# NikhilMukraj/spiking-neural-networks

Measured on AMD Instinct MI355X. Metric: neuron-steps/sec, higher is better.
Workload: dtype f32; 1 GPU; 256x256 Izhikevich lattice, dense gap-junction connectivity (all-to-all, x != y), dt=0.1, weights U[0.5,1.5]; neurons=65536, parallelism=single GPU

## Files before the change

### spiking-neural-networks_amd/csrc/snn_network.hip

```cpp
#include "snn_network_state.hpp"
#include "snn_network_step.hpp"
#include "snn_network_exchange.hpp"
#include "snn_network_verify.hpp"
#include "snn_network_graph.hpp"
#include "snn_network_edge_history.hpp"
#include "snn_network_peaks.hpp"

extern "C" {

int snn_abi_version(void) ABI_TRY { return SNN_ABI_VERSION; } ABI_CATCH
const char *snn_custom_model(void) ABI_TRY { return custom::TYPE_NAME; } ABI_CATCH_PTR
const char *snn_custom_spike_train(void) ABI_TRY { return custom_st::TYPE_NAME; } ABI_CATCH_PTR
const char *snn_custom_refractoriness(void) ABI_TRY { return custom_refr::TYPE_NAME; } ABI_CATCH_PTR
const char *snn_custom_neurotransmitter_kinetics(void) ABI_TRY { return custom_nt::TYPE_NAME; } ABI_CATCH_PTR
const char *snn_custom_receptor_kinetics(void) ABI_TRY { return custom_rc::TYPE_NAME; } ABI_CATCH_PTR
const char *snn_custom_receptors(void) ABI_TRY { return custom_receptors::TYPE_NAME; } ABI_CATCH_PTR
const char *snn_last_error(void) ABI_TRY { return g_last_error.c_str(); } ABI_CATCH_PTR

int snn_network_create(int device, int neuron_model, int nt_kinetics, int receptor_kinetics,
                       int spike_train_model, snn_network_t **out) ABI_TRY
{
    if (!out) return fail(SNN_ERR_BAD_ARG, "out is null");
    *out = nullptr;
    const bool custom_ok = SNN_HAVE_CUSTOM_NEURON && neuron_model == SNN_MODEL_CUSTOM;
    const bool custom_st_ok = SNN_HAVE_CUSTOM_SPIKE_TRAIN && spike_train_model == SNN_ST_CUSTOM;
    const bool custom_nt_ok = SNN_HAVE_CUSTOM_NT && nt_kinetics == SNN_NT_CUSTOM;
    const bool custom_rc_ok = SNN_HAVE_CUSTOM_RC && receptor_kinetics == SNN_RC_CUSTOM;
    if (((neuron_model < 0 || neuron_model > 8) && !custom_ok) || ((nt_kinetics < 0 || nt_kinetics > 3) && !custom_nt_ok) ||
        ((receptor_kinetics < 0 || receptor_kinetics > 2) && !custom_rc_ok) ||
        ((spike_train_model < 0 || spike_train_model > 4) && !custom_st_ok))
        return fail(SNN_ERR_BAD_ARG, "unknown model / kinetics selector");
    int ndev = 0;
    if (hipGetDeviceCount(&ndev) != hipSuccess || ndev <= 0)
        return fail(SNN_ERR_GET_DEVICE, "no HIP device visible");
    if (device < 0 || device >= ndev) return fail(SNN_ERR_GET_DEVICE, "device ordinal out of range");
    HIP_TRY(hipSetDevice(device), SNN_ERR_GET_DEVICE);
    snn_network *net = new snn_network();
    net->device = device;
    for (const OptionRow &r : OPTION_TABLE)
        if (const char *e = r.source != OPTION_ONLY ? getenv(option_env_name(r).c_str()) : nullptr) net->opt.*r.member = option_from_env(r, e);
    net->model = neuron_model; net->nt_kind = nt_kinetics; net->rc_kind = receptor_kinetics;
    net->st_kind = spike_train_model;
    if (const char *e = getenv("SNN_AMD_W24")) net->w24_enabled = !(e[0] == '0' && e[1] == '\0');
    if (hipStreamCreateWithFlags(&net->own_stream, hipStreamNonBlocking) != hipSuccess) {
        delete net;
        return fail(SNN_ERR_QUEUE, "hipStreamCreate failed");
    }
    net->stream = net->own_stream;
    *out = net;
    return SNN_OK;
}
ABI_CATCH

int snn_network_destroy(snn_network_t *net) ABI_TRY
{
    if (!net) return SNN_OK;
    (void)hipSetDevice(net->device);
    if (net->stream) (void)hipStreamSynchronize(net->stream);
    for (auto &e : net->ev_pool) { (void)hipEventDestroy(e.first); (void)hipEventDestroy(e.second); }
    for (auto &e : net->ev_pool_pl) { (void)hipEventDestroy(e.first); (void)hipEventDestroy(e.second); }
    if (net->comm_stream) { (void)hipStreamSynchronize(net->comm_stream); (void)hipStreamDestroy(net->comm_stream); }
    if (net->ev_packed) (void)hipEventDestroy(net->ev_packed);
    if (net->ev_exchanged) (void)hipEventDestroy(net->ev_exchanged);
    if (net->own_stream) (void)hipStreamDestroy(net->own_stream);
    delete net;
    return SNN_OK;
}
ABI_CATCH

static int add_lattice_impl(snn_network_t *net, uint32_t id, uint32_t rows, uint32_t cols, bool st)
{
    if (!net) return fail(SNN_ERR_BAD_ARG, "net is null");
    if (net->finalized) return fail(SNN_ERR_BAD_STATE, "lattices cannot be added after finalize");
    if (find_lattice(net, id))
        return fail(SNN_ERR_BAD_ARG, "lattice id " + std::to_string(id) + " already present");
    if (st && net->st_kind == SNN_ST_NONE) return fail(SNN_ERR_BAD_STATE, "network was created without a spike-train model");
    if ((uint64_t)rows * cols > 0x7FFFFFFFull) return fail(SNN_ERR_DIM_MISMATCH, "lattice too large");
    LatticeInfo l{id, rows, cols, 0, rows * cols, 0, st};
    (st ? net->st_lattices : net->lattices).push_back(l);
    return SNN_OK;
}

int snn_network_add_lattice(snn_network_t *net, uint32_t id, uint32_t rows, uint32_t cols) ABI_TRY
{
    return add_lattice_impl(net, id, rows, cols, false);
}
ABI_CATCH
int snn_network_add_spike_train_lattice(snn_network_t *net, uint32_t id, uint32_t rows, uint32_t cols) ABI_TRY
{
    return add_lattice_impl(net, id, rows, cols, true);
}
ABI_CATCH

static int finalize_impl(snn_network_t *net, int kind, uint32_t post_begin, uint32_t post_end, uint32_t n_shards,
                         uint32_t stride, uint32_t shard_index)
{
    const bool whole = kind == 0;
    if (!net) return fail(SNN_ERR_BAD_ARG, "net is null");
    if (net->finalized) return fail(SNN_ERR_BAD_STATE, "already finalized");
    HIP_TRY(hipSetDevice(net->device), SNN_ERR_GET_DEVICE);
    auto by_id = [](const LatticeInfo &a, const LatticeInfo &b) { return a.id < b.id; };
    std::sort(net->lattices.begin(), net->lattices.end(), by_id);
    std::sort(net->st_lattices.begin(), net->st_lattices.end(), by_id);
    uint64_t off = 0;
    uint32_t slot = 0;
    for (auto &l : net->lattices) { l.first = (uint32_t)off; l.slot = slot++; off += l.count; }
    net->nn = (uint32_t)off;
    slot = 0;
    for (auto &l : net->st_lattices) { l.first = (uint32_t)off; l.slot = slot++; off += l.count; }
    if (off > 0x7FFFFFFFull) return fail(SNN_ERR_DIM_MISMATCH, "network too large");
    net->n_tot = (uint32_t)off;
    net->nc = net->n_tot - net->nn;
    net->n_pad = std::max<uint32_t>(256, round_up(net->nn, 256));
    net->c_pad = std::max<uint32_t>(256, round_up(net->nc, 256));
    if (whole) {
        net->q0 = 0; net->q1 = net->nn;
    } else if (kind == 1) {
        if (post_begin > post_end || post_end > net->nn) return fail(SNN_ERR_DIM_MISMATCH, "shard range outside the population");
        if (stride == 0 || stride % 64 != 0 || n_shards == 0 || (uint64_t)stride * n_shards < net->nn)
            return fail(SNN_ERR_BAD_ARG, "shard stride must be a multiple of 64 covering the population");
        net->q0 = post_begin; net->q1 = post_end;
        net->sharded = true;
        net->n_shards = n_shards; net->shard_stride = stride; net->shard_index = shard_index;
        net->n_pad = std::max<uint32_t>(net->n_pad, round_up(stride * n_shards, 256));
    } else {
        net->q0 = 0; net->q1 = 0;
// ... 891 lines not shown
ABI_CATCH

int snn_set_spike_train_clock(snn_network_t *net, uint32_t id, uint64_t clock) ABI_TRY
{
    if (!net) return fail(SNN_ERR_BAD_ARG, "net is null");
    if (!net->finalized) return fail(SNN_ERR_BAD_STATE, "network not finalized");
    const LatticeInfo *l = find_lattice(net, id);
    if (!l || !l->spike_train) return fail(SNN_ERR_BAD_ARG, "no such spike-train lattice");
    if (clock > 0x7FFFFFFFull) return fail(SNN_ERR_BAD_ARG, "the clock must fit the firing times' 31 bits");
    HIP_TRY(hipSetDevice(net->device), SNN_ERR_GET_DEVICE);
    TRY(end_run(net));
    net->st_clock[l->slot] = (long long)clock;
    return SNN_OK;
}
ABI_CATCH

int snn_get_spike_train_clock(snn_network_t *net, uint32_t id, uint64_t *clock) ABI_TRY
{
    if (!net || !clock) return fail(SNN_ERR_BAD_ARG, "null argument");
    if (!net->finalized) return fail(SNN_ERR_BAD_STATE, "network not finalized");
    const LatticeInfo *l = find_lattice(net, id);
    if (!l || !l->spike_train) return fail(SNN_ERR_BAD_ARG, "no such spike-train lattice");
    HIP_TRY(hipSetDevice(net->device), SNN_ERR_GET_DEVICE);
    TRY(end_run(net));
    *clock = (uint64_t)net->st_clock[l->slot];
    return SNN_OK;
}
ABI_CATCH

const char *snn_debug_verify_report(snn_network_t *net) ABI_TRY { return net ? net->verify_text.c_str() : ""; } ABI_CATCH_PTR

int snn_debug_fail_alloc_at(int64_t n, uint64_t *allocations_so_far) ABI_TRY
{
    AllocFault &f = alloc_fault();
    if (allocations_so_far) *allocations_so_far = f.seen.load(std::memory_order_relaxed);
    f.countdown.store(n > 0 ? n : 0, std::memory_order_relaxed);
    return SNN_OK;
}
ABI_CATCH

int snn_debug_set_host_allocator(snn_host_alloc_fn alloc, snn_host_release_fn release) ABI_TRY
{
    static HostAllocHooks hooks;
    if ((alloc == nullptr) != (release == nullptr)) return fail(SNN_ERR_BAD_ARG, "both functions or none");
    if (!alloc) { host_alloc_hooks().store(nullptr, std::memory_order_release); return SNN_OK; }
    hooks.alloc = alloc; hooks.release = release;
    host_alloc_hooks().store(&hooks, std::memory_order_release);
    return SNN_OK;
}
ABI_CATCH

int snn_debug_checkpoint(snn_network_t *net, int restore) ABI_TRY
{
    if (!net) return fail(SNN_ERR_BAD_ARG, "net is null");
    if (!net->finalized) return fail(SNN_ERR_BAD_STATE, "network not finalized");
    HIP_TRY(hipSetDevice(net->device), SNN_ERR_GET_DEVICE);
    TRY(end_run(net));
    if (restore) net->img_stale = net->img_stale_direct = true;
    if (restore) w24_invalidate(net);
    auto &cp = net->checkpoint;
    hvec<std::pair<void *, size_t>> arrays;
    for (const auto &r : net->registry)
        if (!r.scratch) arrays.emplace_back(r.mem.get(), r.bytes);
    if (net->csr_w) arrays.emplace_back(net->csr_w, (size_t)net->sell_entries * 4);
    if (net->trace) arrays.emplace_back(net->trace, std::max<size_t>(trace_elems(net), 64) * 4);
    for (void *m : {(void *)net->pending, (void *)net->edge_counter})
        if (m) arrays.emplace_back(m, std::max<size_t>(trace_elems(net), 64) * 4);
    size_t total = 0;
    for (const auto &a : arrays) total += a.second;
    if (total > ((size_t)256 << 20)) return fail(SNN_ERR_BAD_STATE, "checkpoints are for small handles (256 MiB of device state at most)");
    const size_t peak_words = (net->want_peaks && net->pk_raster) ? (size_t)net->cur.hist_steps * (net->n_pad / 64) : 0;
    if (!restore) {
        hvec<unsigned long long> peak_rows(peak_words);
        if (peak_words) HIP_TRY(copy_sync(net, peak_rows.data(), net->pk_raster, peak_words * 8, hipMemcpyDeviceToHost), SNN_ERR_BUFFER_READ);
        cp.peak_rows.swap(peak_rows);
        cp.peak_epoch = net->pk_epoch;
        cp.arrays.clear();
        for (const auto &a : arrays) {
            cp.arrays.emplace_back(a.first, hvec<uint8_t>(a.second));
            HIP_TRY(hipMemcpyAsync(cp.arrays.back().second.data(), a.first, a.second, hipMemcpyDeviceToHost, net->stream), SNN_ERR_BUFFER_READ);
        }
        HIP_TRY(hipStreamSynchronize(net->stream), SNN_ERR_WAIT);
        cp.st_clock = net->st_clock; cp.cur = net->cur; cp.cache = net->cache; cp.persistent_run = net->opt.persistent_run;
        cp.valid = true;
        return SNN_OK;
    }
    if (!cp.valid) return fail(SNN_ERR_BAD_STATE, "no checkpoint was taken");
    if (cp.peak_epoch != net->pk_epoch) return fail(SNN_ERR_BAD_STATE, "the handle's structure changed since the checkpoint (peak records switched)");
    std::map<void *, size_t> current(arrays.begin(), arrays.end());
    for (const auto &a : cp.arrays) {
        const auto it = current.find(a.first);
        if (it == current.end() || it->second != a.second.size())
            return fail(SNN_ERR_BAD_STATE, "the handle's structure changed since the checkpoint");
    }
    for (const auto &a : cp.arrays)
        HIP_TRY(hipMemcpyAsync(a.first, a.second.data(), a.second.size(), hipMemcpyHostToDevice, net->stream), SNN_ERR_BUFFER_WRITE);
    HIP_TRY(hipStreamSynchronize(net->stream), SNN_ERR_WAIT);
    if (!cp.peak_rows.empty())
        HIP_TRY(copy_sync(net, net->pk_raster, cp.peak_rows.data(), cp.peak_rows.size() * 8, hipMemcpyHostToDevice), SNN_ERR_BUFFER_WRITE);
    net->st_clock = cp.st_clock; net->cur = cp.cur; net->cache = cp.cache; net->opt.persistent_run = cp.persistent_run;
    net->stdp_pending = false; net->stdp_pending_rows_only = false; net->rstdp_pending = false; net->reward_since_defer = false;
    net->cells_stepped = false; net->local_inputs_done = false; net->run_tag = 1;
    if (net->run_granules) {
        HIP_TRY(hipMemsetAsync(net->run_granules, 0, RUN_GRANULE_WORDS * 8, net->stream), SNN_ERR_BUFFER_WRITE);
        HIP_TRY(hipMemsetAsync(net->run_partials, 0, RUN_PARTIAL_WORDS * 8, net->stream), SNN_ERR_BUFFER_WRITE);
        HIP_TRY(hipStreamSynchronize(net->stream), SNN_ERR_WAIT);
    }
    return SNN_OK;
}
ABI_CATCH

extern "C++" {
namespace {
int run_steps(snn_network *net, uint64_t iterations)
{
    uint64_t it = 0;
    if (iterations >= 4 && net->external_stream && run_resident_shape(net)) net->stat.run_external_stream += 1;
    while (iterations - it >= 4 && run_resident_applies(net)) {
        const uint64_t chunk = std::min<uint64_t>(iterations - it, std::max<uint32_t>(4u, net->opt.run_resident_chunk_steps));
        const RunCursors saved{net->cur, net->stat.run, net->ev_used};
        TRY(run_snapshot(net, false));
        TRY(launch_run_resident(net, chunk, it));
        if (!net->opt.persistent_run) break;
        HIP_TRY(hipStreamSynchronize(net->stream), SNN_ERR_WAIT);
        if (net->run_failed && net->run_failed[0]) {
            net->run_failed[0] = 0u;
            TRY(run_snapshot(net, true));
            HIP_TRY(hipMemsetAsync(net->run_granules, 0, RUN_GRANULE_WORDS * 8, net->stream), SNN_ERR_BUFFER_WRITE);
            HIP_TRY(hipMemsetAsync(net->run_partials, 0, RUN_PARTIAL_WORDS * 8, net->stream), SNN_ERR_BUFFER_WRITE);
            net->run_tag = 1;
            net->cur = saved.cur; net->stat.run = saved.run; net->ev_used = saved.ev_used;
            net->cache.shadow_valid = false;
            net->cache.view_dirty = true;
            net->opt.persistent_run = 0;
            net->stat.run_fallbacks += 1;
            break;
        }
        it += chunk;
    }
    for (; it < iterations; ++it) {
        if (net->nn) TRY(step_begin(net));
        TRY(step_end(net));
        if (net->profile && (net->ev_used >= 8192 || net->ev_used_pl >= 8192)) TRY(collect_profile(net));
    }
    return SNN_OK;
}
}
}

int snn_run(snn_network_t *net, uint64_t iterations) ABI_TRY
{
    if (!net) return fail(SNN_ERR_BAD_ARG, "net is null");
    if (!net->finalized) return fail(SNN_ERR_BAD_STATE, "network not finalized");
    if (net->n_shards > 1) return fail(SNN_ERR_BAD_STATE, "sharded handles are stepped with snn_step_begin/end or snn_run_sharded");
    if (iterations == 0 || net->n_tot == 0) return SNN_OK;
    if (!net->electrical && !net->chemical) return SNN_OK;
    HIP_TRY(hipSetDevice(net->device), SNN_ERR_GET_DEVICE);
    TRY(begin_run(net, iterations));
    TRY(verify_applies(net) ? run_verified(net, iterations) : run_steps(net, iterations));
    return end_run(net, true);
}
ABI_CATCH

int snn_step_begin_local(snn_network_t *net) ABI_TRY
{
    if (!net) return fail(SNN_ERR_BAD_ARG, "net is null");
    if (!net->finalized) return fail(SNN_ERR_BAD_STATE, "network not finalized");
    if (!net->electrical && !net->chemical) return SNN_OK;
    HIP_TRY(hipSetDevice(net->device), SNN_ERR_GET_DEVICE);
    TRY(begin_run(net, 1));
    if (net->interior_pending) return step_interior(net);
    if (net->nn && !net->csr && !net->any_plasticity && !net->any_modulation && !net->drive_threshold && !net->local_inputs_done) {
        TRY(launch_inputs(net, INPUTS_LOCAL));
        net->local_inputs_done = true;
    }
    return SNN_OK;
}
ABI_CATCH

// ... 830 lines not shown
```

### spiking-neural-networks_amd/csrc/snn_network_state.hpp

```cpp
#pragma once
#include <hip/hip_runtime.h>

#include <algorithm>
#include <atomic>
#include <chrono>
#include <cmath>
#include <cstdint>
#include <cstdio>
#include <cstdlib>
#include <cstring>
#include <map>
#include <memory>
#include <new>
#include <stdexcept>
#include <string>
#include <utility>
#include <vector>

#include "../../include/snn_amd.h"
#include "snn_kernels_connect.hpp"
#include "snn_kernels_connect_csr.hpp"
#include "snn_kernels_csr.hpp"
#include "snn_kernels_dense_step.hpp"
#include "snn_kernels_edge_history.hpp"
// ... 205 lines not shown
    bool reward_since_defer = false;

    uint32_t nn = 0, nc = 0, n_tot = 0, n_pad = 0, c_pad = 0;
    uint32_t q0 = 0, q1 = 0, n_loc = 0, ld = 0, n_chunks = 0;
    XLayout xl{0};
    bool sharded = false;
    uint32_t n_shards = 1, shard_index = 0, shard_stride = 0;
    bool block_mode = false;
    hvec<uint32_t> lattice_slab;
    hvec<std::pair<uint32_t, uint32_t>> ranges;
    uint32_t n_owned = 0;
    hvec<uint32_t> owned_local_host;
    hvec<uint32_t> local_row_host;
    dev_ptr<uint32_t> own_block_dev, local_row_dev;
    dev_ptr<unsigned long long> own_mask_dev;
    RowMap rowmap{};
    bool x_dirty = true;
    bool x_agreed = false;
    bool refresh_agreed = false;
    int x_mode = SNN_EXCHANGE_ALLGATHER;
    uint32_t x_planes = 0, x_plane_id[WIRE_MAX_PLANES] = {0, 0, 0, 0};
    uint64_t x_block_words = 0;
    uint32_t *wire = nullptr;
    size_t wire_words = 0;
    hvec<hvec<uint32_t>> halo_need, halo_send;
    bool halo_committed = false;
    dev_ptr<uint32_t> halo_send_buf, halo_recv_buf, halo_send_idx, halo_recv_idx;
    hvec<uint64_t> x_send_off, x_send_words, x_recv_off, x_recv_words;
    dev_ptr<uint32_t> seg_count_dev[2], seg_first_dev[2];
    dev_ptr<uint64_t> seg_offset_dev[2], seg_loff_dev[2];
    uint32_t seg_n[2] = {0, 0}, seg_max[2] = {0, 0};
    dev_ptr<uint32_t> csr_border_dev, csr_interior_dev;
    uint32_t n_border = 0, n_interior = 0;
    dev_ptr<uint32_t> pack_ptr_dev, pack_segoff_dev, pack_count_dev, pack_index_dev;
    uint32_t recv_total = 0, send_bitmap_words = 0;
    bool send_bits_clean = true;
    bool update_packed = false;
    bool step_packed = false;
    bool interior_pending = false;
    dev_ptr<uint32_t> halo_send_buf2, halo_recv_buf2;
    dev_ptr<uint32_t> csr_plan_direct, halo_word_dev;
    bool direct_capable = false;
    bool peer_capable = false;
    bool direct_run = false;
    int hx_par = 0;
    bool stamp_pending = false;
    bool tail_done = false;
    dev_ptr<unsigned long long> p2p_recv[2];
    dev_ptr<uint32_t> p2p_flags;
    dev_ptr<uint32_t> p2p_done_blocks;
    pinned_ptr<uint32_t> p2p_failed;
    dev_ptr<uint32_t> agree_words_dev;
    uint32_t agree_words_cap = 0;
    uint64_t p2p_recv_words = 0;
    struct P2pPeer { uint64_t recv[2] = {0, 0}, flags = 0, recv_offset = 0; bool set = false; };
    hvec<P2pPeer> p2p_peers;
    dev_ptr<unsigned long long *> p2p_dst_dev[2];
    dev_ptr<uint32_t> p2p_peer_dev;
    dev_ptr<uint32_t *> p2p_signal_dev;
    uint32_t p2p_n_signal = 0;
    bool p2p_connected = false;
    hvec<dev_ptr<void>> p2p_retired;
    bool peer_run = false;
    uint32_t p2p_epoch = 0;
    hipStream_t comm_stream = nullptr;
    hipEvent_t ev_packed = nullptr, ev_exchanged = nullptr;

    struct Registered { dev_ptr<void> mem; size_t bytes; bool scratch; };
    hvec<Registered> registry;
    uint64_t registry_generation = 0;
    bool csr = false;
    uint64_t nnz = 0;
    dev_ptr<uint32_t> csr_ptr, csr_pre, csr_post, csr_t_ptr, csr_t_edge;
    dev_ptr<uint32_t> csr_row_len, csr_edge_slot;
    dev_ptr<float> csr_w;
    uint64_t sell_entries = 0;
    hvec<uint32_t> edge_slot_host;
    float *W = nullptr;
    dev_ptr<uint32_t> w24, w24_range;
    uint32_t w24_base = 0;
    bool w24_valid = false;
    bool w24_refused = false;
    bool w24_enabled = true;
    float *xbuf = nullptr;
    float *part_i = nullptr, *part_t = nullptr;
    uint32_t *n_in = nullptr, *tcount = nullptr;
    NeuronArrays na{};
    CellArrays ca{};
    uint32_t *lattice_slot = nullptr;
    float *stdp_dev = nullptr;
    uint32_t *plast_dev = nullptr;
    uint32_t *spike_list = nullptr, *spike_count = nullptr;
    hvec<uint32_t> cell_list_host;
    dev_ptr<uint32_t> cell_list_dev;
    uint32_t n_cells_listed = 0;
    dev_ptr<uint32_t> csr_plan;
    dev_ptr<uint32_t> csr_img_hdr, csr_plan_win;
    dev_ptr<uint4> csr_img_rec;
    uint64_t img_records = 0, img_staged_slices = 0;
    bool img_stale = true;
    dev_ptr<uint32_t> csr_img_hdr_direct, csr_plan_win_direct;
    dev_ptr<uint4> csr_img_rec_direct;
    uint64_t img_staged_slices_direct = 0;
    bool img_stale_direct = true;
    hvec<uint32_t> sell_pre_host, slice_ptr_host;
    uint2 *cell_view[2] = {nullptr, nullptr};
    bool cells_stepped = false;
    UniformTable *uni_neuron = nullptr, *uni_cell = nullptr;
    unsigned long long *run_granules = nullptr;
    unsigned long long *run_partials = nullptr;
    uint32_t run_tag = 1;
    float *run_w_out = nullptr;
    pinned_ptr<uint32_t> run_failed;
    uint32_t run_probed_grid = 0;
    CopyEntry *snap_table = nullptr;
    uint32_t *snap_buf = nullptr;
    uint32_t snap_entries = 0, snap_max_words = 0;
    uint64_t snap_registry_seen = 0;
    size_t snap_words = 0;
    hvec<CopyEntry> snap_table_host;
    size_t verify_words = 0;
    uint32_t *verify_buf = nullptr;
    dev_ptr<uint32_t> verify_report;
    pinned_ptr<char> copy_stage;
    dev_ptr<uint32_t> verify_third;
    size_t verify_third_words = 0;
    dev_ptr<char> verify_big;
    size_t verify_big_bytes = 0;
    uint64_t snap_generation = 0;
    std::string verify_text;
    struct Checkpoint {
        bool valid = false;
        hvec<std::pair<void *, hvec<uint8_t>>> arrays;
        hvec<long long> st_clock;
        Cursors cur;
        CacheState cache;
        uint32_t persistent_run = 1;
        hvec<unsigned long long> peak_rows;
        uint64_t peak_epoch = 0;
    } checkpoint;
    unsigned long long *run_timing = nullptr;
    unsigned long long run_timing_last[4] = {0, 0, 0, 0};
    uint32_t run_timing_steps = 0;
    bool stdp_pending = false;
    bool stdp_pending_rows_only = false;
    uint32_t *stdp_rowbits = nullptr;
    uint32_t *stdp_flag = nullptr;
    float *stdp_dcol = nullptr, *stdp_drow = nullptr;
    uint32_t dcol_stride = 0;
    long long *st_clock_dev = nullptr;
    pinned_ptr<long long> st_clock_pinned;
    bool run_active = false;
    float *shadow[2] = {nullptr, nullptr};
    uint32_t *tile_done = nullptr;
    uint32_t tile_done_len = 0;
    bool local_inputs_done = false;

    std::map<std::string, Attr> neuron_attrs, cell_attrs;

    int want_vhist = 0, want_raster = 0;
    int want_avg = 0, want_eeg = 0, want_counts = 0;
    hvec<int> want_whist;
    hvec<dev_ptr<float>> whist;
    bool any_whist = false;
    hvec<uint32_t> eh_slot;
    uint32_t eh_n1 = 0, eh_n2 = 0, eh_first2 = 0, eh_ld = 0;
    dev_ptr<uint32_t> eh_pre, eh_post;
    dev_ptr<unsigned long long> eh_offset;
    dev_ptr<float> eh_hist;
    hvec<uint2> pk_cfg_host;
    dev_ptr<uint2> pk_cfg;
    bool want_peaks = false;
    float *pk_prev = nullptr;
    uint32_t *pk_left = nullptr;
    dev_ptr<unsigned long long> pk_raster;
    uint64_t pk_epoch = 0;
    float eeg_ref = 0.007f, eeg_dist = 0.8f, eeg_cond = 251.0f;
    dev_ptr<float> summ_avg, summ_eeg;
    uint32_t *spike_counts = nullptr, *lat_first_dev = nullptr, *lat_count_dev = nullptr;
    uint64_t hist_cap = 0;
    hvec<hvec<float>> preset_host;
    dev_ptr<float> preset_times_dev;
    uint32_t hist_every = 1;
    dev_ptr<float> vhist, st_vhist;
    dev_ptr<unsigned long long> raster;

    uint64_t drive_seed = 0;
    uint32_t drive_threshold = 0;
    float drive_voltage = 0.0f;
    hvec<std::pair<hipEvent_t, hipEvent_t>> ev_pool_pl;
    size_t ev_used_pl = 0;
    uint64_t prof_launches_pl = 0;
    double prof_ms_pl = 0.0;
    int profile = 0;
    hvec<std::pair<hipEvent_t, hipEvent_t>> ev_pool;
    hvec<int> ev_counts;
    size_t ev_used = 0;
    uint64_t prof_launches = 0;
    double prof_ms = 0.0;
};

namespace {
static_assert(Options{}.run_resident_spin_limit == RUN_RESIDENT_SPIN_LIMIT, "snn_options.hpp restates the kernel header's default");

struct StatRow { const char *name; uint64_t (*read)(const snn_network &); };
#define STAT(field) [](const snn_network &n) -> uint64_t { return n.field; }
const StatRow STAT_TABLE[] = {
    {"persistent_run_launches", STAT(stat.run.launches)},
    {"persistent_run_steps", STAT(stat.run.steps)},
    {"persistent_run_stdp_steps", STAT(stat.run.stdp_steps)},
    {"persistent_run_fallbacks", STAT(stat.run_fallbacks)},
    {"persistent_run_external_stream", STAT(stat.run_external_stream)},
    {"halo_direct_steps", STAT(stat.direct_steps)},
    {"halo_peer_steps", STAT(stat.peer_steps)},
    {"steps_dense_one_launch", STAT(stat.steps_dense_one_launch)},
    {"steps_dense_close", STAT(stat.steps_dense_close)},
// ... 749 lines not shown
```

### spiking-neural-networks_amd/csrc/snn_network_step.hpp

```cpp
#pragma once
#include "snn_dispatch.hpp"
#include "snn_network_state.hpp"

namespace {

enum ProfilePool { PROFILE_GRAPH_PASS, PROFILE_PLASTICITY };
int profile_open(snn_network *net, ProfilePool which, int passes, hipEvent_t *e1)
{
    *e1 = nullptr;
    if (!net->profile) return SNN_OK;
    auto &pool = which == PROFILE_PLASTICITY ? net->ev_pool_pl : net->ev_pool;
    size_t &used = which == PROFILE_PLASTICITY ? net->ev_used_pl : net->ev_used;
    if (used == pool.size()) {
        hipEvent_t x, y;
        HIP_TRY(hipEventCreate(&x), SNN_ERR_QUEUE);
        HIP_TRY(hipEventCreate(&y), SNN_ERR_QUEUE);
        pool.emplace_back(x, y);
    }
    if (which == PROFILE_GRAPH_PASS) {
        net->ev_counts.resize(pool.size(), 1);
        net->ev_counts[used] = passes;
    }
    const auto ev = pool[used++];
    *e1 = ev.second;
// ... 443 lines not shown
    if (net->n_loc == 0 || net->nn == 0) { net->stdp_pending_rows_only = false; return SNN_OK; }
    StdpArgs a = stdp_args(net);
    const unsigned sy = 64;
    if (net->stdp_pending_rows_only) {
        net->stdp_pending_rows_only = false;
    } else {
        hipLaunchKernelGGL(k_stdp_apply_columns, dim3((net->n_tot + 255) / 256, sy), dim3(256), 0, net->stream, a);
        HIP_TRY(hipGetLastError(), SNN_ERR_QUEUE);
    }
    hipLaunchKernelGGL(k_stdp_apply_rows, dim3((net->n_loc + 255) / 256, sy), dim3(256), 0, net->stream, a);
    HIP_TRY(hipGetLastError(), SNN_ERR_QUEUE);
    return SNN_OK;
}

int flush_rstdp(snn_network *net)
{
    if (!net->rstdp_pending) return SNN_OK;
    net->rstdp_pending = false;
    return launch_rstdp_pass(net, net->reward_since_defer ? RM_DOPAMINE_BEFORE : RM_DOPAMINE);
}

int time_input_pass(snn_network *net, float *ms)
{
    *ms = 0.0f;
    hipEvent_t e0 = nullptr, e1 = nullptr;
    if (hipEventCreate(&e0) != hipSuccess || hipEventCreate(&e1) != hipSuccess) return fail(SNN_ERR_QUEUE, "hipEventCreate failed");
    const size_t bytes = (size_t)net->n_tot * net->ld * 4;
    const int passes = bytes < ((size_t)4 << 30) ? 8 : 1;
    int rc = launch_inputs(net);
    if (rc == SNN_OK && hipEventRecord(e0, net->stream) != hipSuccess) rc = fail(SNN_ERR_QUEUE, "hipEventRecord failed");
    for (int i = 0; i < passes && rc == SNN_OK; ++i) rc = launch_inputs(net);
    if (rc == SNN_OK && (hipEventRecord(e1, net->stream) != hipSuccess || hipEventSynchronize(e1) != hipSuccess ||
                         hipEventElapsedTime(ms, e0, e1) != hipSuccess))
        rc = fail(SNN_ERR_WAIT, "placement timing failed");
    *ms /= (float)passes;
    (void)hipEventDestroy(e0);
    (void)hipEventDestroy(e1);
    return rc;
}

int choose_matrix_placement(snn_network *net)
{
    const size_t count = net->csr ? 0 : wcount(net->n_tot, net->ld);
    const size_t bytes = count * sizeof(float);
    if (bytes >= ((size_t)1 << 30) && net->n_loc) {
        const int prof = net->profile;
        net->profile = 0;
        float best_ms = 0.0f;
        int rc = time_input_pass(net, &best_ms);
        hvec<dev_ptr<void>> losers;
        for (int cand = 0; cand < 4 && rc == SNN_OK; ++cand) {
            size_t free_b = 0, total_b = 0;
            dev_ptr<void> b;
            if (hipMemGetInfo(&free_b, &total_b) != hipSuccess || free_b < bytes + (bytes >> 2) ||
                alloc_streamed(&b, bytes) != hipSuccess)
                break;
            float *a = net->W;
            float ms_b = 0.0f;
            net->W = static_cast<float *>(b.get());
            rc = time_input_pass(net, &ms_b);
            if (getenv("SNN_DEBUG_PLACEMENT"))
                fprintf(stderr, "[snn] matrix placement: held %p %.3f ms, candidate %p %.3f ms\n", (void *)a, best_ms, b.get(), ms_b);
            if (rc == SNN_OK && ms_b < best_ms * 0.99f) {
                losers.push_back(dev_replace(net, a, std::move(b)));
                w24_invalidate(net);
                best_ms = ms_b;
            } else {
                net->W = a;
                losers.push_back(std::move(b));
            }
        }
        net->profile = prof;
        if (rc != SNN_OK) return rc;
    }
    if (count) {
        hipLaunchKernelGGL(k_fill_u32, dim3(4096), dim3(256), 0, net->stream,
                           reinterpret_cast<uint32_t *>(net->W), count, 0x7FC00000u);
        HIP_TRY(hipGetLastError(), SNN_ERR_QUEUE);
        HIP_TRY(hipStreamSynchronize(net->stream), SNN_ERR_WAIT);
    }
    return SNN_OK;
}

int ensure_w24(snn_network *net)
{
    if (!w24_applies(net)) {
        net->w24 = nullptr;
        w24_invalidate(net);
        return SNN_OK;
    }
    if (net->w24_valid || net->w24_refused) return SNN_OK;
    auto refuse = [&]() { (void)hipGetLastError(); net->w24 = nullptr; net->w24_refused = true; return SNN_OK; };
    if (!net->w24_range && snn_malloc(&net->w24_range, 256) != hipSuccess) return refuse();
    uint32_t range[2] = {0xFFFFFFFFu, 0u};
    HIP_TRY(copy_sync(net, net->w24_range, range, 8, hipMemcpyHostToDevice), SNN_ERR_BUFFER_WRITE);
    hipLaunchKernelGGL(k_w24_range, dim3(4096), dim3(256), 0, net->stream, net->W, net->ld, net->n_loc, net->n_tot, net->w24_range.get());
    HIP_TRY(hipGetLastError(), SNN_ERR_QUEUE);
    HIP_TRY(copy_sync(net, range, net->w24_range, 8, hipMemcpyDeviceToHost), SNN_ERR_BUFFER_READ);
    if (!w24_encodable(range[0], range[1])) return refuse();
    const size_t bytes = w24_image_bytes(net->n_tot, net->ld);
    if (!net->w24 && alloc_streamed(&net->w24, bytes) != hipSuccess) return refuse();
    net->w24_base = w24_base(range[0], range[1]);
    hipLaunchKernelGGL(k_w24_pack, dim3((net->ld + 255) / 256, (unsigned)w24_row_units(net->n_tot)), dim3(256), 0, net->stream,
                       net->W, net->ld, net->n_loc, net->n_tot, net->w24_base, reinterpret_cast<w24_v4u *>(net->w24.get()));
    HIP_TRY(hipGetLastError(), SNN_ERR_QUEUE);
    net->w24_valid = true;
    if (bytes >= ((size_t)1 << 30)) {
        const int prof = net->profile;
        net->profile = 0;
        float best_ms = 0.0f;
        int rc = time_input_pass(net, &best_ms);
        hvec<dev_ptr<uint32_t>> losers;
        for (int cand = 0; cand < 2 && rc == SNN_OK; ++cand) {
            size_t free_b = 0, total_b = 0;
            dev_ptr<uint32_t> b;
            if (hipMemGetInfo(&free_b, &total_b) != hipSuccess || free_b < bytes + (bytes >> 2) || alloc_streamed(&b, bytes) != hipSuccess) {
                (void)hipGetLastError();
                break;
            }
            if (hipMemcpyAsync(b, net->w24, bytes, hipMemcpyDeviceToDevice, net->stream) != hipSuccess) { losers.push_back(std::move(b)); break; }
            std::swap(net->w24, b);
            float ms_b = 0.0f;
            rc = time_input_pass(net, &ms_b);
            if (getenv("SNN_DEBUG_PLACEMENT"))
                fprintf(stderr, "[snn] image placement: held %p %.3f ms, candidate %p %.3f ms\n", (void *)b.get(), best_ms, (void *)net->w24.get(), ms_b);
            if (rc == SNN_OK && ms_b < best_ms * 0.99f) best_ms = ms_b;
            else std::swap(net->w24, b);
            losers.push_back(std::move(b));
        }
        net->profile = prof;
        if (rc != SNN_OK) return rc;
    }
    return SNN_OK;
}

bool fused_step_applies(const snn_network *net)
{
    return fused_step_possible(net) && !net->local_inputs_done;
}

int fused_step_args(snn_network *net, InputsArgs &a, UpdateArgs &u, bool in_place = false)
{
    const size_t xelems = (size_t)NUM_PLANES * net->xl.stride;
    if (in_place) {
        net->cache.shadow_valid = false;
    } else if (!net->shadow[0]) {
        TRY(dev_alloc_t(net, &net->shadow[0], xelems));
        TRY(dev_alloc_t(net, &net->shadow[1], xelems));
        net->cache.shadow_valid = false;
    }
    if (!in_place && !net->cache.shadow_valid) {
        for (int i = 0; i < 2; ++i)
            HIP_TRY(hipMemcpyAsync(net->shadow[i], net->xbuf, xelems * 4, hipMemcpyDeviceToDevice, net->stream),
                    SNN_ERR_BUFFER_WRITE);
        net->cache.shadow_valid = true;
        net->stat.shadow_refreshes += 1;
    }
    float *cur = in_place ? net->xbuf : net->shadow[net->cache.shadow_cur];
    float *next = in_place ? nullptr : net->shadow[net->cache.shadow_cur ^ 1];
    a = InputsArgs{};
    a.chunk_first = 0; a.hole_begin = net->n_chunks; a.hole_count = 0;
    a.W = net->W; a.ld = net->ld; a.n_loc = net->n_loc; a.q0 = net->q0; a.rows = net->rowmap; a.n_neurons = net->nn; a.n_tot = net->n_tot;
    a.xbuf = cur; a.xl = net->xl; a.gap_conductance = net->na.gap_conductance; a.uni = net->uni_neuron;
    a.st_value = net->ca.presyn_value; a.st_last_firing_time = net->ca.last_firing_time;
    a.st_view = net->cell_view[net->cache.cell_view_cur];
    a.st_nt_t = net->ca.nt_t; a.st_nt_flags = net->ca.nt_flags; a.c_pad = net->c_pad;
    a.nt_flags = net->na.nt_flags; a.n_pad = net->n_pad;
    a.part_i = net->part_i; a.part_t = net->part_t; a.n_chunks = net->n_chunks;
    for (int k = 0; k < K_TYPES; ++k) a.live_type[k] = (uint32_t)k;
    u = UpdateArgs{};
    u.n = net->na;
    u.n.xbuf = cur;
    u.part_i = net->part_i; u.part_t = net->part_t; u.n_in = net->n_in; u.tcount = net->tcount;
    u.ld = net->ld; u.n_chunks = net->n_chunks; u.q0 = net->q0; u.n_loc = net->n_loc; u.rows = net->rowmap;
    u.clock = net->cur.clock;
    u.electrical = net->electrical; u.chemical = net->chemical; u.nt_kind = net->nt_kind; u.rc_kind = net->rc_kind;
    u.vhist_row = (record_now(net) && net->want_vhist && net->vhist) ? net->vhist + (size_t)net->cur.hist_steps * net->n_pad : nullptr;
    u.spike_row = (record_now(net) && net->want_raster && net->raster) ? net->raster + (size_t)net->cur.hist_steps * (net->n_pad / 64) : nullptr;
    u.spike_counts = net->want_counts ? net->spike_counts : nullptr;
    u.xout = net->xbuf; u.xout2 = next;
    u.has_nt = net->any_nt_neurons ? 1 : 0;
    u.live_mask = net->cache.live_mask_applied;
    u.bcm = net->model == SNN_MODEL_BCM_IZHIKEVICH;
    u.model_is_custom = net->model == SNN_MODEL_CUSTOM;
    return SNN_OK;
}

int launch_step_resident(snn_network *net)
{
    ResidentArgs r{};
    TRY(fused_step_args(net, r.in, r.up));
    hipEvent_t e1 = nullptr;
    TRY(profile_open(net, PROFILE_GRAPH_PASS, 1, &e1));
    const bool quarters = net->opt.resident_quarters && net->n_chunks <= 2 && net->n_tot > 64;
    const dim3 grid((net->n_loc + 63) / 64), block(64 * net->n_chunks * (quarters ? 4 : 1));
    for_model(ResidentStepModels{}, net->model, [&](auto M) {
        for_synapses(net->electrical, net->chemical, [&](auto E, auto C) {
            if (quarters) hipLaunchKernelGGL((k_step_resident_q<M(), E(), C()>), grid, block, 0, net->stream, r);
            else hipLaunchKernelGGL((k_step_resident<M(), E(), C()>), grid, block, 0, net->stream, r);
        });
    });
    HIP_TRY(hipGetLastError(), SNN_ERR_QUEUE);
    TRY(profile_close(net, e1));
    net->cache.shadow_cur ^= 1;
    return SNN_OK;
}

bool dense_close_applies(const snn_network *net)
{
    return !SNN_HAVE_CUSTOM_MODEL && net->opt.dense_close && !net->csr && !net->sharded && !net->drive_threshold && net->n_loc && net->n_tot &&
           net->n_loc == net->nn && net->electrical && matrix_streamed(net) && !net->local_inputs_done && !net->stdp_pending &&
           !net->rstdp_pending && net->opt.input_shape == 0 && net->n_chunks <= net->opt.dense_close_max_chunks;
}

// ... 673 lines not shown
```

### spiking-neural-networks_amd/csrc/snn_w24.hpp

```cpp
#pragma once
#include <cstddef>
#include <cstdint>

#if defined(__HIPCC__) || defined(__CUDACC__)
#define SNN_W24_HD __host__ __device__
#else
#define SNN_W24_HD
#endif

namespace snn {

constexpr uint32_t W24_ABSENT = 0xFFFFFFu;
constexpr uint32_t W24_MAX_SPAN = 0xFFFFFEu;
constexpr uint32_t W24_UNIT_ROWS = 16, W24_UNIT_COLS = 64;
constexpr size_t W24_PLANE_BYTES = 1024, W24_UNIT_BYTES = 3 * W24_PLANE_BYTES;
constexpr size_t W24_SLACK = 16 * W24_UNIT_BYTES;

SNN_W24_HD inline bool w24_encodable(uint32_t min_bits, uint32_t max_bits)
{
    return min_bits > max_bits || max_bits - min_bits <= W24_MAX_SPAN;
}
SNN_W24_HD inline uint32_t w24_base(uint32_t min_bits, uint32_t max_bits) { return min_bits > max_bits ? 0u : min_bits; }

SNN_W24_HD inline uint32_t w24_encode(uint32_t bits, uint32_t base) { return bits - base; }
SNN_W24_HD inline bool w24_present(uint32_t code) { return code != W24_ABSENT; }
SNN_W24_HD inline uint32_t w24_decode(uint32_t code, uint32_t base) { return code + base; }

SNN_W24_HD inline size_t w24_row_units(uint32_t n_rows) { return ((size_t)n_rows + W24_UNIT_ROWS - 1) / W24_UNIT_ROWS; }
SNN_W24_HD inline size_t w24_image_bytes(uint32_t n_rows, size_t ld)
{
    return w24_row_units(n_rows) * (ld / W24_UNIT_COLS) * W24_UNIT_BYTES + W24_SLACK;
}
SNN_W24_HD inline size_t w24_unit_offset(size_t ru, size_t cb, size_t ld) { return (ru * (ld / W24_UNIT_COLS) + cb) * W24_UNIT_BYTES; }
SNN_W24_HD inline size_t w24_byte_index(uint32_t p, uint32_t q, size_t ld, uint32_t k = 0)
{
    const uint32_t in_lane = 3u * (p % W24_UNIT_ROWS) + k;
    return w24_unit_offset(p / W24_UNIT_ROWS, q / W24_UNIT_COLS, ld) + (size_t)(in_lane / 16u) * W24_PLANE_BYTES +
           (size_t)(q % W24_UNIT_COLS) * 16u + in_lane % 16u;
}

SNN_W24_HD inline void w24_pack16(const uint32_t (&code)[16], uint32_t (&dw)[12])
{
    for (int d = 0; d < 12; ++d) dw[d] = 0u;
    for (int r = 0; r < 16; ++r)
        for (int k = 0; k < 3; ++k) {
            const int byte = 3 * r + k;
            dw[byte >> 2] |= ((code[r] >> (8 * k)) & 0xFFu) << (8 * (byte & 3));
        }
}
SNN_W24_HD inline uint32_t w24_unpack(const uint32_t (&dw)[12], int r)
{
    uint32_t c = 0;
    for (int k = 0; k < 3; ++k) {
        const int byte = 3 * r + k;
        c |= ((dw[byte >> 2] >> (8 * (byte & 3))) & 0xFFu) << (8 * k);
    }
    return c;
}

}
```

Before: 31.87 million neuron-steps/s.

## Place the 24-bit weight image in W's original allocation region

For large dense matrices, the float weight matrix W is copied into a fresh allocation and the packed 24-bit weight image takes over W's original device region. The placement choice is timed against a fresh allocation using a median of three passes, and the faster placement is kept. The aim is to put the hot image in a physical region that gives better memory bandwidth for the input pass. In exchange it adds a full-matrix device copy at setup, checkpoint pointer remapping, and the logic to move W back when the image is released.

```diff
diff --git a/spiking-neural-networks_amd/csrc/snn_network.hip b/spiking-neural-networks_amd/csrc/snn_network.hip
--- a/spiking-neural-networks_amd/csrc/snn_network.hip
+++ b/spiking-neural-networks_amd/csrc/snn_network.hip
@@ -42,6 +42,8 @@
     net->model = neuron_model; net->nt_kind = nt_kinetics; net->rc_kind = receptor_kinetics;
     net->st_kind = spike_train_model;
     if (const char *e = getenv("SNN_AMD_W24")) net->w24_enabled = !(e[0] == '0' && e[1] == '\0');
+    if (const char *e = getenv("SNN_AMD_W24_REGION")) net->w24_region_enabled = !(e[0] == '0' && e[1] == '\0');
+    if (const char *e = getenv("SNN_AMD_W24_REGION_MIN")) net->w24_region_min = std::min<size_t>(net->w24_region_min, strtoull(e, nullptr, 0));
     if (hipStreamCreateWithFlags(&net->own_stream, hipStreamNonBlocking) != hipSuccess) {
         delete net;
         return fail(SNN_ERR_QUEUE, "hipStreamCreate failed");
@@ -1099,19 +1101,21 @@
         }
         HIP_TRY(hipStreamSynchronize(net->stream), SNN_ERR_WAIT);
         cp.st_clock = net->st_clock; cp.cur = net->cur; cp.cache = net->cache; cp.persistent_run = net->opt.persistent_run;
+        cp.matrix = net->W;
         cp.valid = true;
         return SNN_OK;
     }
     if (!cp.valid) return fail(SNN_ERR_BAD_STATE, "no checkpoint was taken");
     if (cp.peak_epoch != net->pk_epoch) return fail(SNN_ERR_BAD_STATE, "the handle's structure changed since the checkpoint (peak records switched)");
+    auto now_at = [&](void *then) { return (then && then == cp.matrix) ? (void *)net->W : then; };
     std::map<void *, size_t> current(arrays.begin(), arrays.end());
     for (const auto &a : cp.arrays) {
-        const auto it = current.find(a.first);
+        const auto it = current.find(now_at(a.first));
         if (it == current.end() || it->second != a.second.size())
             return fail(SNN_ERR_BAD_STATE, "the handle's structure changed since the checkpoint");
     }
     for (const auto &a : cp.arrays)
-        HIP_TRY(hipMemcpyAsync(a.first, a.second.data(), a.second.size(), hipMemcpyHostToDevice, net->stream), SNN_ERR_BUFFER_WRITE);
+        HIP_TRY(hipMemcpyAsync(now_at(a.first), a.second.data(), a.second.size(), hipMemcpyHostToDevice, net->stream), SNN_ERR_BUFFER_WRITE);
     HIP_TRY(hipStreamSynchronize(net->stream), SNN_ERR_WAIT);
     if (!cp.peak_rows.empty())
         HIP_TRY(copy_sync(net, net->pk_raster, cp.peak_rows.data(), cp.peak_rows.size() * 8, hipMemcpyHostToDevice), SNN_ERR_BUFFER_WRITE);
diff --git a/spiking-neural-networks_amd/csrc/snn_network_state.hpp b/spiking-neural-networks_amd/csrc/snn_network_state.hpp
--- a/spiking-neural-networks_amd/csrc/snn_network_state.hpp
+++ b/spiking-neural-networks_amd/csrc/snn_network_state.hpp
@@ -311,6 +311,9 @@
     bool w24_valid = false;
     bool w24_refused = false;
     bool w24_enabled = true;
+    bool w24_in_region = false;
+    bool w24_region_enabled = true;
+    size_t w24_region_min = (size_t)1 << 30;
     float *xbuf = nullptr;
     float *part_i = nullptr, *part_t = nullptr;
     uint32_t *n_in = nullptr, *tcount = nullptr;
@@ -361,6 +364,7 @@
     struct Checkpoint {
         bool valid = false;
         hvec<std::pair<void *, hvec<uint8_t>>> arrays;
+        void *matrix = nullptr;
         hvec<long long> st_clock;
         Cursors cur;
         CacheState cache;
diff --git a/spiking-neural-networks_amd/csrc/snn_network_step.hpp b/spiking-neural-networks_amd/csrc/snn_network_step.hpp
--- a/spiking-neural-networks_amd/csrc/snn_network_step.hpp
+++ b/spiking-neural-networks_amd/csrc/snn_network_step.hpp
@@ -549,15 +549,75 @@
     return SNN_OK;
 }
 
+int time_image_pass(snn_network *net, float *ms)
+{
+    float t[3] = {0.0f, 0.0f, 0.0f};
+    for (float &x : t) TRY(time_input_pass(net, &x));
+    std::sort(t, t + 3);
+    *ms = t[1];
+    return SNN_OK;
+}
+
+bool w24_hand_over(snn_network *net)
+{
+    const size_t wbytes = dev_bytes(net, net->W);
+    size_t free_b = 0, total_b = 0;
+    dev_ptr<void> b;
+    if (!wbytes || hipMemGetInfo(&free_b, &total_b) != hipSuccess || free_b < wbytes + (wbytes >> 2) || alloc_streamed(&b, wbytes) != hipSuccess) {
+        (void)hipGetLastError();
+        return false;
+    }
+    const auto t0 = std::chrono::steady_clock::now();
+    if (hipMemcpyAsync(b.get(), net->W, wbytes, hipMemcpyDeviceToDevice, net->stream) != hipSuccess ||
+        hipStreamSynchronize(net->stream) != hipSuccess) {
+        (void)hipGetLastError();
+        return false;
+    }
+    float *const moved = static_cast<float *>(b.get());
+    dev_ptr<void> region = dev_replace(net, net->W, std::move(b));
+    if (!region) return false;
+    if (getenv("SNN_DEBUG_PLACEMENT"))
+        fprintf(stderr, "[snn] image region: W moves out of %p to %p, %.3f ms; the image takes W's region\n", region.get(), (void *)moved,
+                std::chrono::duration<double, std::milli>(std::chrono::steady_clock::now() - t0).count());
+    net->W = moved;
+    net->w24.reset(static_cast<uint32_t *>(region.release()));
+    net->w24_in_region = true;
+    return true;
+}
+
+int w24_return_region(snn_network *net, dev_ptr<uint32_t> region)
+{
+    const size_t wbytes = dev_bytes(net, net->W);
+    const auto t0 = std::chrono::steady_clock::now();
+    HIP_TRY(hipMemcpyAsync(region.get(), net->W, wbytes, hipMemcpyDeviceToDevice, net->stream), SNN_ERR_BUFFER_WRITE);
+    HIP_TRY(hipStreamSynchronize(net->stream), SNN_ERR_WAIT);
+    float *const back = reinterpret_cast<float *>(region.get());
+    const void *const left = net->W;
+    dev_replace(net, net->W, dev_ptr<void>(region.release()));
+    net->W = back;
+    net->w24_in_region = false;
+    if (getenv("SNN_DEBUG_PLACEMENT"))
+        fprintf(stderr, "[snn] image region: W moves back from %p into its region %p, %.3f ms\n", left, (void *)back,
+                std::chrono::duration<double, std::milli>(std::chrono::steady_clock::now() - t0).count());
+    return SNN_OK;
+}
+
+int w24_release(snn_network *net)
+{
+    if (net->w24_in_region) TRY(w24_return_region(net, std::move(net->w24)));
+    net->w24 = nullptr;
+    return SNN_OK;
+}
+
 int ensure_w24(snn_network *net)
 {
     if (!w24_applies(net)) {
-        net->w24 = nullptr;
+        TRY(w24_release(net));
         w24_invalidate(net);
         return SNN_OK;
     }
     if (net->w24_valid || net->w24_refused) return SNN_OK;
-    auto refuse = [&]() { (void)hipGetLastError(); net->w24 = nullptr; net->w24_refused = true; return SNN_OK; };
+    auto refuse = [&]() { (void)hipGetLastError(); net->w24_refused = true; return w24_release(net); };
     if (!net->w24_range && snn_malloc(&net->w24_range, 256) != hipSuccess) return refuse();
     uint32_t range[2] = {0xFFFFFFFFu, 0u};
     HIP_TRY(copy_sync(net, net->w24_range, range, 8, hipMemcpyHostToDevice), SNN_ERR_BUFFER_WRITE);
@@ -566,19 +626,27 @@
     HIP_TRY(copy_sync(net, range, net->w24_range, 8, hipMemcpyDeviceToHost), SNN_ERR_BUFFER_READ);
     if (!w24_encodable(range[0], range[1])) return refuse();
     const size_t bytes = w24_image_bytes(net->n_tot, net->ld);
+    const bool kept = net->w24.get() != nullptr;
+    bool handed_over = false;
+    if (!kept &&net->w24_region_enabled && bytes >= net->w24_region_min && w24_fits_matrix(net->n_tot, net->ld) &&
+        bytes <= dev_bytes(net, net->W))
+        handed_over = w24_hand_over(net);
     if (!net->w24 && alloc_streamed(&net->w24, bytes) != hipSuccess) return refuse();
     net->w24_base = w24_base(range[0], range[1]);
     hipLaunchKernelGGL(k_w24_pack, dim3((net->ld + 255) / 256, (unsigned)w24_row_units(net->n_tot)), dim3(256), 0, net->stream,
                        net->W, net->ld, net->n_loc, net->n_tot, net->w24_base, reinterpret_cast<w24_v4u *>(net->w24.get()));
     HIP_TRY(hipGetLastError(), SNN_ERR_QUEUE);
     net->w24_valid = true;
-    if (bytes >= ((size_t)1 << 30)) {
+    if (getenv("SNN_DEBUG_PLACEMENT") && kept)
+        fprintf(stderr, "[snn] image placement: packed again into %p (%s)\n", (void *)net->w24.get(), net->w24_in_region ? "W's region" : "fresh");
+    if (handed_over || (!net->w24_in_region && bytes >= ((size_t)1 << 30))) {
         const int prof = net->profile;
         net->profile = 0;
         float best_ms = 0.0f;
-        int rc = time_input_pass(net, &best_ms);
+        int rc = time_image_pass(net, &best_ms);
         hvec<dev_ptr<uint32_t>> losers;
-        for (int cand = 0; cand < 2 && rc == SNN_OK; ++cand) {
+        dev_ptr<uint32_t> region;
+        for (int cand = 0; cand < (handed_over ? 1 : 2) && rc == SNN_OK; ++cand) {
             size_t free_b = 0, total_b = 0;
             dev_ptr<uint32_t> b;
             if (hipMemGetInfo(&free_b, &total_b) != hipSuccess || free_b < bytes + (bytes >> 2) || alloc_streamed(&b, bytes) != hipSuccess) {
@@ -588,15 +656,28 @@
             if (hipMemcpyAsync(b, net->w24, bytes, hipMemcpyDeviceToDevice, net->stream) != hipSuccess) { losers.push_back(std::move(b)); break; }
             std::swap(net->w24, b);
             float ms_b = 0.0f;
-            rc = time_input_pass(net, &ms_b);
+            rc = time_image_pass(net, &ms_b);
             if (getenv("SNN_DEBUG_PLACEMENT"))
-                fprintf(stderr, "[snn] image placement: held %p %.3f ms, candidate %p %.3f ms\n", (void *)b.get(), best_ms, (void *)net->w24.get(), ms_b);
-            if (rc == SNN_OK && ms_b < best_ms * 0.99f) best_ms = ms_b;
-            else std::swap(net->w24, b);
+                fprintf(stderr, "[snn] image placement: held %p (%s) %.3f ms, candidate %p (fresh) %.3f ms\n", (void *)b.get(),
+                        handed_over ? "W's region" : "fresh", best_ms, (void *)net->w24.get(), ms_b);
+            if (rc == SNN_OK && ms_b < best_ms * 0.99f) {
+                best_ms = ms_b;
+                if (handed_over) { region = std::move(b); continue; }
+            } else {
+                std::swap(net->w24, b);
+            }
             losers.push_back(std::move(b));
         }
         net->profile = prof;
+        if (rc == SNN_OK && hipStreamSynchronize(net->stream) != hipSuccess) rc = fail(SNN_ERR_WAIT, "image placement search failed");
+        if (region) {
+            const int rc_back = w24_return_region(net, std::move(region));
+            if (rc == SNN_OK) rc = rc_back;
+        }
         if (rc != SNN_OK) return rc;
+        if (getenv("SNN_DEBUG_PLACEMENT"))
+            fprintf(stderr, "[snn] image placement: the image stays in %p (%s), %.3f ms\n", (void *)net->w24.get(),
+                    net->w24_in_region ? "W's region" : "fresh", best_ms);
     }
     return SNN_OK;
 }
diff --git a/spiking-neural-networks_amd/csrc/snn_w24.hpp b/spiking-neural-networks_amd/csrc/snn_w24.hpp
--- a/spiking-neural-networks_amd/csrc/snn_w24.hpp
+++ b/spiking-neural-networks_amd/csrc/snn_w24.hpp
@@ -31,6 +31,11 @@
 {
     return w24_row_units(n_rows) * (ld / W24_UNIT_COLS) * W24_UNIT_BYTES + W24_SLACK;
 }
+SNN_W24_HD inline size_t w24_matrix_body_bytes(uint32_t n_rows, size_t ld) { return (((size_t)n_rows + 3) / 4) * 4 * ld * 4; }
+SNN_W24_HD inline bool w24_fits_matrix(uint32_t n_rows, size_t ld)
+{
+    return ld >= W24_UNIT_COLS && ld % W24_UNIT_COLS == 0 && w24_image_bytes(n_rows, ld) <= w24_matrix_body_bytes(n_rows, ld);
+}
 SNN_W24_HD inline size_t w24_unit_offset(size_t ru, size_t cb, size_t ld) { return (ru * (ld / W24_UNIT_COLS) + cb) * W24_UNIT_BYTES; }
 SNN_W24_HD inline size_t w24_byte_index(uint32_t p, uint32_t q, size_t ld, uint32_t k = 0)
 {
```

Result: faster. 34.29 million neuron-steps/s, median of 6 (+7.6%).
